# nekopanda/Amatsukaze

Measured on NVIDIA H100. Metric: 1920x1080i YV12 frames/sec (logo-eval + combing), higher is better.
Workload: dtype u8+f32

## Files before the change

amatsukaze_b200/csrc/amtk_b200.cu:

```cuda
#include "amtk_internal.h"
#include "logo_kernels.cuh"
#include "comb_kernels.cuh"
#include "comb_stream.cuh"
#include "comb_mma.cuh"
#include "scan_kernels.cuh"
#include "tnr_kernels.cuh"
#include <algorithm>
#include <cfloat>
#include <cmath>
#include <cstdlib>
#include <cstring>
#include <deque>
#include <memory>
#include <mutex>
#include <type_traits>

extern "C" { static int logo_ensure_device(const amtk_logo* cl, amtk_ctx* ctx, bool need_tables); }

namespace amtk {

static thread_local std::string g_error;
static constexpr size_t kEvalSmemLimit = 226 * 1024;
void set_error(const std::string& msg) { g_error = msg; }
bool cuda_ok(cudaError_t e, const char* what) {
// ... 272 lines not shown
          job.scores, count, countPad, n, sp.nfades, hl.blackScore, sp.take_abs, sum_out, out_frame_stride, sp.out_off, sp.out_fade_stride, rows);
    } else {
      logo_sum_kernel<<<(total + kSumThreads - 1) / kSumThreads, kSumThreads, 0, st>>>(
          job.scores, count, countPad, n, sp.nfades, hl.blackScore, sp.take_abs, sum_out, out_frame_stride, sp.out_off, sp.out_fade_stride, rows);
    }
    AMTK_CUDA(cudaGetLastError());
    ctx->launches += 2;
  }
  return 1;
}

static bool roi_inside(const amtk::HostLogo& full, const amtk_clip* clip, int pitch_elems) {
  if (full.imgx < 0 || full.imgy < 0) return false;
  const long long last = (long long)full.imgx + full.w - 1 + (long long)(full.imgy + full.h - 1) * pitch_elems;
  const long long plane_elems = (long long)clip->pitch_y / clip->bytes_per_sample * clip->height;
  return full.imgx + full.w <= pitch_elems && last < plane_elems;
}

static int comb_thresholds_ok(const amtk_comb_params* p, int bytes_per_sample) {
  if (bytes_per_sample == 2) {
    const int all[6] = { p->th_move_y, p->th_shima_y, p->th_lshima_y, p->th_move_c, p->th_shima_c, p->th_lshima_c };
    for (int v : all) if (v < 1) { set_error("comb: thresholds must be >= 1"); return 0; }
    if (p->th_move_y > 32768 || p->th_move_c > 32768) { set_error("comb: th_move must be in [1,32768] for 16-bit samples"); return 0; }
    return 1;
  }
  const int m[2] = { p->th_move_y, p->th_move_c };
  const int s[4] = { p->th_shima_y, p->th_lshima_y, p->th_shima_c, p->th_lshima_c };
  for (int v : m) if (v < 1 || v > 128) { set_error("comb: th_move must be in [1,128]"); return 0; }
  for (int v : s) if (v < 1 || v > 2047) { set_error("comb: th_shima/th_lshima must be in [1,2047]"); return 0; }
  return 1;
}

struct CombVariant {
  int R, strip, stages, sync, TH, boxH, threads, smem;
  void (*kernel)(const CombArgs);
  void (*kernel16)(const CombArgs);
};
template <typename Cfg> static CombVariant make_variant() {
  return CombVariant{ Cfg::R, Cfg::STRIP, Cfg::STAGES, Cfg::SYNC, Cfg::TH, Cfg::BOXH, Cfg::THREADS, Cfg::SMEM, comb_tma_kernel<Cfg, 1>, nullptr };
}
template <typename Cfg> static CombVariant make_variant16() {
  return CombVariant{ Cfg::R, Cfg::STRIP, Cfg::STAGES, Cfg::SYNC, Cfg::TH, Cfg::BOXH, Cfg::THREADS, Cfg::SMEM, comb_tma_kernel<Cfg, 1>, comb_tma_kernel<Cfg, 2> };
}
static const CombVariant* comb_variants(int* n) {
  static const CombVariant v[] = {
    make_variant16<CombCfg<15, 8, 3, 0>>(), make_variant16<CombCfg<16, 8, 3, 0>>(), make_variant16<CombCfg<17, 8, 3, 0>>(),
    make_variant<CombCfg<17, 8, 2, 0>>(), make_variant<CombCfg<17, 8, 4, 0>>(), make_variant<CombCfg<17, 8, 3, 1>>(),
  };
  *n = (int)(sizeof(v) / sizeof(v[0]));
  return v;
}

static int pick_comb_R(int hY, int hC) {
  int best = 16; long long best_waste = -1;
  for (int R = 17; R >= 15; --R) {
    const int th = 8 * R;
    const long long waste = (long long)((hY + th - 1) / th) * th - hY + 2LL * (((hC + th - 1) / th) * th - hC) / 2;
    if (best_waste < 0 || waste < best_waste) { best_waste = waste; best = R; }
  }
  return best;
}

struct WsVariant { int R, stages, warps, bps, TH, boxH, smem; bool band; void (*kernel)(const WsArgs); };
template <typename Cfg> static WsVariant make_ws() { return WsVariant{ Cfg::R, Cfg::STAGES, Cfg::WARPS, Cfg::BPS, Cfg::TH, Cfg::BOXH, Cfg::SMEM, Cfg::BAND, comb_ws_kernel<Cfg> }; }
static const WsVariant* ws_variants(int* n) {
  static const WsVariant v[] = { make_ws<WsCfg<17, 2>>(), make_ws<WsCfg<15, 2>>(), make_ws<WsCfg<16, 2>>(), make_ws<WsCfg<9, 2>>(), make_ws<WsCfg<15, 3>>(), make_ws<WsCfg<12, 2>>(), make_ws<WsCfg<10, 2>>(),
                                 make_ws<WsCfg<15, 2, 7>>(), make_ws<WsCfg<13, 2, 5>>(), make_ws<WsCfg<15, 2, 2>>(), make_ws<WsCfg<15, 3, 3>>(),
                                 make_ws<WsCfg<15, 2, 4, 2>>(), make_ws<WsCfg<16, 2, 4, 2>>(), make_ws<WsCfg<17, 2, 4, 2>>(),
                                 make_ws<WbCfg<15, 2>>(), make_ws<WbCfg<16, 2>>(), make_ws<WbCfg<17, 2>>(), make_ws<WbCfg<15, 3>>(),
                                 make_ws<WtCfg<15, 2>>(), make_ws<WtCfg<16, 2>>() };
  *n = (int)(sizeof(v) / sizeof(v[0]));
  return v;
}
static int pick_ws_R(int hY, int hC, int runs = kWsRuns) {
  int best = 17; long long best_waste = -1;
  for (int R : { 17, 16, 15 }) {
    const int th = runs * R;
    const long long waste = 2LL * ((long long)((hY + th - 1) / th) * th - hY) + 2LL * ((long long)((hC + th - 1) / th) * th - hC);
    if (best_waste < 0 || waste < best_waste) { best_waste = waste; best = R; }
  }
  return best;
}

static int ws_watchdog_ok(amtk_ctx* ctx) {
  if (!ctx->watch_pending) return 1;
  AMTK_CUDA(cudaEventSynchronize(ctx->ev_watch));
  ctx->watch_pending = false;
  const int* d = ctx->ws_watch;
  if (d[0]) {
    char msg[256];
    snprintf(msg, sizeof(msg), "comb_ws (band form): a device-side wait of the previous launch timed out (wait %d, step %d, CTA %d, thread %d, parity %d); its counters are not valid",
             d[1], d[2], d[3], d[4], d[5]);
    AMTK_FAIL(msg);
  }
  return 1;
}

static const int* ws_watch_record(const amtk_ctx* ctx) {
  return ctx->plan.dev.at<const int>(ctx->plan.q_off) + 16;
}

static CUtensorMapL2promotion comb_l2_promotion(const amtk_ctx* ctx) {
  switch (ctx->knobs.comb_l2) {
    case 0: return CU_TENSOR_MAP_L2_PROMOTION_NONE;
    case 64: return CU_TENSOR_MAP_L2_PROMOTION_L2_64B;
    case 256: return CU_TENSOR_MAP_L2_PROMOTION_L2_256B;
    default: return CU_TENSOR_MAP_L2_PROMOTION_L2_128B;
  }
}

template <typename Launch>
static int comb_launch(amtk_ctx* ctx, int* counts, int nf, Launch launch) {
  AMTK_CUDA(cudaMemsetAsync(counts, 0, (size_t)nf * 12 * sizeof(int), ctx->stream));
  std::pair<EventHandle, EventHandle> ev;
  if (ctx->timing) {
    if (!ctx->timing_pool.empty()) { ev = std::move(ctx->timing_pool.back()); ctx->timing_pool.pop_back(); }
    else { AMTK_CUDA(cudaEventCreate(ev.first.put())); AMTK_CUDA(cudaEventCreate(ev.second.put())); }
    AMTK_CUDA(cudaEventRecord(ev.first, ctx->stream));
  }
  launch();
  AMTK_CUDA(cudaGetLastError());
  if (ctx->timing) { AMTK_CUDA(cudaEventRecord(ev.second, ctx->stream)); ctx->timing_events.push_back(std::move(ev)); }
  ctx->launches += 1;
  return 1;
}

static_assert(std::has_unique_object_representations<amtk_ctx::CombPlanKey>::value, "plan keys are compared with memcmp");

template <typename Build>
static int comb_plan(amtk_ctx* ctx, const amtk_ctx::CombPlanKey& key, WsArgs& args, Build build) {
  amtk_ctx::CombPlan& plan = ctx->plan;
  if (!plan.valid || memcmp(&plan.key, &key, sizeof(key)) != 0) {
    const std::vector<CombSegment> segs = build();
    const size_t seg_bytes = segs.size() * sizeof(CombSegment);
    plan.q_off = (seg_bytes + 255) & ~(size_t)255;
    plan.valid = false;
    if (!plan.dev.ensure(plan.q_off + 256)) return 0;
    AMTK_CUDA(cudaMemcpyAsync(plan.dev.at(), segs.data(), seg_bytes, cudaMemcpyHostToDevice, ctx->stream));
    AMTK_CUDA(cudaStreamSynchronize(ctx->stream));
    plan.nitems = (int)segs.size(); plan.key = key; plan.valid = true;
  }
  AMTK_CUDA(cudaMemsetAsync(plan.dev.at(plan.q_off), 0, 256, ctx->stream));
  args.segs = plan.dev.at<const CombSegment>();
  args.nitems = plan.nitems;
  args.queue = plan.dev.at<int>(plan.q_off);
  return 1;
}

static const WsVariant* ws_variant(const amtk_ctx* ctx, const amtk_clip* clip, bool tall = true) {
  const int hY = clip->height, hC = clip->height >> clip->log_uvy;
  int nvar = 0; const WsVariant* vars = ws_variants(&nvar);
  const int bps = clip->bytes_per_sample;
  const bool band = bps == 1 && ctx->knobs.comb_ws_band && ctx->knobs.comb_ws_warps == kWsWarps;
  auto find = [&](int runs, int warps) -> const WsVariant* {
    const int R = ctx->knobs.comb_R ? ctx->knobs.comb_R : pick_ws_R(hY, hC, runs);
    for (int i = 0; i < nvar; ++i)
      if (vars[i].R == R && vars[i].stages == ctx->knobs.comb_ws_stages && vars[i].warps == warps && vars[i].bps == bps && vars[i].band == band) return &vars[i];
    return nullptr;
  };
  if (band && tall && ctx->knobs.comb_ws_band == 2)
    if (const WsVariant* V = find(kWtGroups * kWsRuns, kWtGroups * kWsWarps)) return V;
  return find(kWsRuns, ctx->knobs.comb_ws_warps);
}

static int launch_comb_ws(amtk_ctx* ctx, const amtk_clip* clip, const Window& win, int lo, int hi,
                          const amtk_comb_params* prm, int* dcounts, int out_row0, const ScanItemJob* lj = nullptr) {
  const int hY = clip->height, hC = clip->height >> clip->log_uvy;
  const int wY = clip->width, wC = clip->width >> clip->log_uvx;
  const int bps = clip->bytes_per_sample;
  const WsVariant* V = ws_variant(ctx, clip);
  if (!V) AMTK_FAIL("comb: no warp-stream kernel variant for the requested AMTK_COMB_* settings");
  const bool band = V->band;
  if (lj && !band) AMTK_FAIL("comb: logo items need the band form");
  const int WW = V->warps;
  if (!ws_watchdog_ok(ctx)) return 0;
  WsArgs args;
  memset(&args, 0, sizeof(args));
  const CUtensorMapL2promotion promo = comb_l2_promotion(ctx);
  for (int pl = 0; pl < 3; ++pl) {
    const long long off = pl == 0 ? 0 : (pl == 1 ? clip->off_u : clip->off_v);
    cuuint64_t gdim[3] = { (cuuint64_t)(pl ? wC : wY) * bps, (cuuint64_t)(pl ? hC : hY), (cuuint64_t)win.count };
    cuuint64_t gstr[2] = { (cuuint64_t)(pl ? clip->pitch_uv : clip->pitch_y), (cuuint64_t)clip->frame_stride };
    cuuint32_t box[3] = { (cuuint32_t)(band ? kWbHalf : kWsTW), (cuuint32_t)V->boxH, 1u };
    if (encode_map(ctx, &args.map[pl], CU_TENSOR_MAP_DATA_TYPE_UINT8, 3, win.dev_base + off, gdim, gstr, box, CU_TENSOR_MAP_SWIZZLE_NONE, promo) != CUDA_SUCCESS)
      AMTK_FAIL("cuTensorMapEncodeTiled failed");
  }
  const int remC = (wC * bps) % kWsTW;
  const long long uv_dist = clip->off_v - clip->off_u;
  const bool pair_uv = !band && ctx->knobs.comb_merge_uv && remC > 0 && remC <= kWsTW / 2 && uv_dist > 0 && (uv_dist & 15) == 0;
  if (pair_uv) {
    cuuint64_t gdim[4] = { (cuuint64_t)wC * bps, 2u, (cuuint64_t)hC, (cuuint64_t)win.count };
    cuuint64_t gstr[3] = { (cuuint64_t)uv_dist, (cuuint64_t)clip->pitch_uv, (cuuint64_t)clip->frame_stride };
    cuuint32_t box[4] = { (cuuint32_t)(kWsTW / 2), 2u, (cuuint32_t)V->boxH, 1u };
    if (encode_map(ctx, &args.map_uv, CU_TENSOR_MAP_DATA_TYPE_UINT8, 4, win.dev_base + clip->off_u, gdim, gstr, box, CU_TENSOR_MAP_SWIZZLE_NONE, promo) != CUDA_SUCCESS)
      AMTK_FAIL("cuTensorMapEncodeTiled(uv pair) failed");
  }
  const int tyY = (hY + V->TH - 1) / V->TH, tyC = (hC + V->TH - 1) / V->TH;
  int tile0 = 0, nc = 0;
  auto thresholds = [&](WsClass& C, bool chroma) {
    C.cls = chroma ? 1 : 0; C.H = chroma ? hC : hY;
    const int tM = chroma ? prm->th_move_c : prm->th_move_y, tS = chroma ? prm->th_shima_c : prm->th_shima_y, tL = chroma ? prm->th_lshima_c : prm->th_lshima_y;
    if (bps == 1) {
      C.thM = (unsigned)(0x80 - tM) * 0x01010101u;
      C.thS = (unsigned)tS * 0x00010001u;
      C.thL = (unsigned)tL * 0x00010001u;
    } else {
      C.thM = (unsigned)std::min(tM, 2047) * 0x00010001u;
      C.thS = (unsigned)(8192 + std::min(tS, 8191)) * 0x00010001u;
      C.thL = (unsigned)(8192 + std::min(tL, 8191)) * 0x00010001u;
    }
  };
  for (int pl = 0; pl < 3; ++pl) {
    WsClass& C = args.cl[nc];
    const int w = (pl ? wC : wY) * bps;
    C.kind = 0; C.map = pl; C.W = w; thresholds(C, pl != 0);
    C.tilesX = band ? (w + kWbW - 1) / kWbW : (pl && pair_uv) ? w / kWsTW : (w + kWsTW - 1) / kWsTW;
    C.tile0 = tile0; C.ntiles = C.tilesX * (pl ? tyC : tyY);
    if (C.ntiles == 0) continue;
    tile0 += C.ntiles; ++nc;
  }
  if (pair_uv) {
    WsClass& C = args.cl[nc];
    C.kind = 1; C.x0 = wC * bps - remC; C.tilesX = 1; thresholds(C, true);
    C.tile0 = tile0; C.ntiles = tyC; tile0 += C.ntiles; ++nc;
  }
  args.nclasses = nc;
  const int ntiles = tile0, nf = hi - lo;
  amtk_ctx::CombPlan& plan = ctx->plan;
  if (plan.occ_kernel != (const void*)V->kernel) {
    int occ = 0;
    AMTK_CUDA(cudaFuncSetAttribute(V->kernel, cudaFuncAttributeMaxDynamicSharedMemorySize, V->smem));
    AMTK_CUDA(cudaOccupancyMaxActiveBlocksPerMultiprocessor(&occ, V->kernel, 32 * WW, V->smem));
    if (occ < 1) AMTK_FAIL("comb kernel does not fit on an SM");
    plan.occ = occ; plan.occ_kernel = (const void*)V->kernel;
  }
  int occ = plan.occ;
  if (ctx->knobs.comb_ctas > 0) occ = std::min(occ, ctx->knobs.comb_ctas);
  const int logoF = lj ? lj->frames : 0, nlogo = lj ? (nf + logoF - 1) / logoF : 0;
  const long long total = (long long)ntiles * nf + nlogo;
  const int per_cta = band ? 1 : WW;
  const int nwarps = ctx->sm_count * occ * per_cta;
  const int grid = (int)std::min<long long>((long long)ctx->sm_count * occ, (total + per_cta - 1) / per_cta);
  const int f0 = lo - win.first;
  const amtk_ctx::CombPlanKey key{ (const void*)V->kernel, wY, hY, wC, hC, ntiles, nf, f0, ctx->knobs.comb_item, ctx->knobs.comb_tail,
                                   occ * WW, nlogo, logoF };
  if (!comb_plan(ctx, key, args, [&] {
    int big = ctx->knobs.comb_item > 0 ? ctx->knobs.comb_item : 64, small = std::max(4, big / 4);
    while (big > 8 && (long long)ntiles * (nf / big) < 6LL * nwarps) { big /= 2; small = std::max(4, big / 4); }
    const int tail_frames = std::min(nf, std::max(small, (int)(nf * 0.15)));
    const int head_frames = nf - tail_frames;
    const int tiny = ctx->knobs.comb_tail;
    const int end_frames = (tiny > 0 && tiny < small) ? std::min(tail_frames, std::max(tiny, (int)(nf * 0.04))) : 0;
    const int mid_end = nf - end_frames;
    std::vector<CombSegment> segs;
    segs.reserve((size_t)ntiles * (head_frames / big + tail_frames / small + (tiny > 0 ? end_frames / tiny : 0) + 3) + nlogo);
    auto tier = [&](int fa, int fz, int step) {
      if (band) {
        for (int f = fa; f < fz; f += step)
          for (int t = 0; t < ntiles; ++t) segs.push_back(CombSegment{ t, f0 + f, f0 + std::min(fz, f + step) });
      } else {
        for (int t = 0; t < ntiles; ++t)
          for (int f = fa; f < fz; f += step) segs.push_back(CombSegment{ t, f0 + f, f0 + std::min(fz, f + step) });
      }
    };
    tier(0, head_frames, big);
    if (nlogo > 0) {
      const std::vector<CombSegment> head(segs);
      const long long nhead = (long long)head.size();
      segs.clear();
      int k = 0;
      for (long long i = 0; i <= nhead; ++i) {
        for (; k < nlogo && (2LL * k + 1) * nhead / (2LL * nlogo) <= i; ++k)
          segs.push_back(CombSegment{ -1, f0 + k * logoF, f0 + std::min(nf, (k + 1) * logoF) });
        if (i < nhead) segs.push_back(head[(size_t)i]);
      }
    }
    tier(head_frames, mid_end, small);
    if (tiny > 0) tier(mid_end, nf, tiny);
    return segs;
  }))
    return 0;
  args.counts = dcounts;
  args.out_frame0 = out_row0 - win.first;
  args.prefetch = ctx->knobs.comb_ws_prefetch;
  if (lj) args.logo = *lj;
  if (!comb_launch(ctx, dcounts + (size_t)(lo - out_row0) * 12, nf, [&] { V->kernel<<<grid, 32 * WW, V->smem, ctx->stream>>>(args); }))
    return 0;
  if (band) {
    if (!ctx->ws_watch) {
      AMTK_CUDA(cudaHostAlloc(ctx->ws_watch.put(), 8 * sizeof(int), cudaHostAllocDefault));
      AMTK_CUDA(cudaEventCreateWithFlags(ctx->ev_watch.put(), cudaEventDisableTiming));
    }
    AMTK_CUDA(cudaMemcpyAsync(ctx->ws_watch, ws_watch_record(ctx), 8 * sizeof(int), cudaMemcpyDeviceToHost, ctx->stream));
    AMTK_CUDA(cudaEventRecord(ctx->ev_watch, ctx->stream));
    ctx->watch_pending = true;
  }
  return 1;
}

static int launch_comb_mma(amtk_ctx* ctx, const amtk_clip* clip, const Window& win, int lo, int hi,
                           const amtk_comb_params* prm, int* dcounts, int out_row0) {
  const int hY = clip->height, hC = clip->height >> clip->log_uvy;
  const int wY = clip->width, wC = clip->width >> clip->log_uvx;
  WsArgs args;
  memset(&args, 0, sizeof(args));
  for (int pl = 0; pl < 3; ++pl) {
    const long long off = pl == 0 ? 0 : (pl == 1 ? clip->off_u : clip->off_v);
    cuuint64_t gdim[3] = { (cuuint64_t)(pl ? wC : wY), (cuuint64_t)(pl ? hC : hY), (cuuint64_t)win.count };
    cuuint64_t gstr[2] = { (cuuint64_t)(pl ? clip->pitch_uv : clip->pitch_y), (cuuint64_t)clip->frame_stride };
    cuuint32_t box[3] = { (cuuint32_t)kMmTW, (cuuint32_t)kMmBoxH, 1u };
    if (encode_map(ctx, &args.map[pl], CU_TENSOR_MAP_DATA_TYPE_UINT8, 3, win.dev_base + off, gdim, gstr, box, CU_TENSOR_MAP_SWIZZLE_128B,
                   comb_l2_promotion(ctx)) != CUDA_SUCCESS)
      AMTK_FAIL("cuTensorMapEncodeTiled failed");
  }
  const int tyY = (hY + kMmTH - 1) / kMmTH, tyC = (hC + kMmTH - 1) / kMmTH;
  int tile0 = 0, nc = 0;
  for (int pl = 0; pl < 3; ++pl) {
    WsClass& C = args.cl[nc];
    const bool chroma = pl != 0;
    C.kind = 0; C.map = pl; C.cls = chroma ? 1 : 0; C.H = chroma ? hC : hY;
    C.thM = (unsigned)(0x80 - (chroma ? prm->th_move_c : prm->th_move_y)) * 0x01010101u;
    C.thS = (unsigned)(chroma ? prm->th_shima_c : prm->th_shima_y) * 0x00010001u;
    C.thL = (unsigned)(chroma ? prm->th_lshima_c : prm->th_lshima_y) * 0x00010001u;
    C.tilesX = ((chroma ? wC : wY) + kMmTW - 1) / kMmTW;
    C.tile0 = tile0; C.ntiles = C.tilesX * (chroma ? tyC : tyY);
    if (C.ntiles == 0) continue;
    tile0 += C.ntiles; ++nc;
  }
  args.nclasses = nc;
  const int ntiles = tile0, nf = hi - lo;
  amtk_ctx::CombPlan& plan = ctx->plan;
  const int NS = ctx->knobs.comb_mma == 2 ? 2 : 1;
  void (*kern)(const WsArgs) = NS == 2 ? comb_mma_kernel<2> : comb_mma_kernel<1>;
  const int smem = NS * kMmSmemPerStream + kMmBandBytes + 1024;
  if (plan.occ_kernel != (const void*)kern) {
    AMTK_CUDA(cudaFuncSetAttribute(kern, cudaFuncAttributeMaxDynamicSharedMemorySize, smem));
    int occ_q = 0;
    AMTK_CUDA(cudaOccupancyMaxActiveBlocksPerMultiprocessor(&occ_q, kern, kMmThreads, smem));
    if (occ_q < 1) AMTK_FAIL("comb_mma: kernel does not fit on an SM");
    plan.occ = occ_q; plan.occ_kernel = (const void*)kern;
  }
  int occ = plan.occ;
  if (ctx->knobs.comb_ctas > 0) occ = std::min(occ, ctx->knobs.comb_ctas);
  const int npairs_t = (ntiles + NS - 1) / NS;
  const long long total = (long long)npairs_t * nf;
  const int nstreams = ctx->sm_count * occ;
  const int grid = (int)std::min<long long>(nstreams, total);
  const int f0 = lo - win.first;
  const amtk_ctx::CombPlanKey key{ (const void*)kern, wY, hY, wC, hC, ntiles, nf, f0, ctx->knobs.comb_item, 0, occ, 0, 0 };
  if (!comb_plan(ctx, key, args, [&] {
    int big = ctx->knobs.comb_item > 0 ? ctx->knobs.comb_item : 64, small = std::max(4, big / 4);
    while (big > 8 && (long long)npairs_t * (nf / big) < 6LL * nstreams) { big /= 2; small = std::max(4, big / 4); }
    const int tail_frames = std::min(nf, std::max(small, (int)(nf * 0.15)));
    const int head_frames = nf - tail_frames;
    std::vector<CombSegment> segs;
    segs.reserve((size_t)NS * npairs_t * (head_frames / big + tail_frames / small + 2));
    auto push_block = [&](int fa, int fz) {
      for (int t = 0; t < ntiles; t += NS) {
        segs.push_back(CombSegment{ t, fa, fz });
        if (NS == 2) segs.push_back(CombSegment{ t + 1 < ntiles ? t + 1 : ~t, fa, fz });
      }
    };
    for (int f = 0; f < head_frames; f += big) push_block(f0 + f, f0 + std::min(head_frames, f + big));
    for (int f = head_frames; f < nf; f += small) push_block(f0 + f, f0 + std::min(nf, f + small));
    return segs;
  }))
    return 0;
  args.counts = dcounts;
  args.out_frame0 = out_row0 - win.first;
  if (!comb_launch(ctx, dcounts + (size_t)(lo - out_row0) * 12, nf, [&] { kern<<<grid, kMmThreads, smem, ctx->stream>>>(args); }))
    return 0;
  int dbg[8] = { 0, 0, 0, 0, 0, 0, 0, 0 };
  AMTK_CUDA(cudaMemcpyAsync(dbg, args.queue + 16, sizeof(dbg), cudaMemcpyDeviceToHost, ctx->stream));
  AMTK_CUDA(cudaStreamSynchronize(ctx->stream));
  if (dbg[0]) {
    char msg[256];
    snprintf(msg, sizeof(msg), "comb_mma<%d>: a device-side wait timed out (wait %d, step %d, CTA %d, thread %d, parity %d); results discarded",
             NS, dbg[1], dbg[2], dbg[3], dbg[4], dbg[5]);
    AMTK_FAIL(msg);
  }
// ... 840 lines not shown
  if (!(ctx->knobs.eval_par && n <= 16 && ctx->side_stream && ctx->side_stream2))
    return launch_eval(ctx, clip, win, lo, hi, pitch, sp, dout, 33, row0, ctx->stream, 0, frame_list) &&
           launch_eval(ctx, clip, win, lo, hi, pitch, st, dout, 33, row0, ctx->stream, 0, frame_list) &&
           launch_eval(ctx, clip, win, lo, hi, pitch, sb, dout, 33, row0, ctx->stream, 0, frame_list);
  const EvalSpec* specs[3] = { &sp, &st, &sb };
  size_t off[3], total = 0;
  for (int i = 0; i < 3; ++i) {
    if (!logo_ensure_device(specs[i]->logo, ctx, true)) return 0;
    off[i] = total;
    total += (((size_t)n * 11 * specs[i]->logo->countPad * sizeof(float)) + 255) & ~(size_t)255;
  }
  if (!ctx->scratch.ensure(total)) return 0;
  cudaStream_t streams[3] = { ctx->stream, ctx->side_stream, ctx->side_stream2 };
  cudaEvent_t joins[3] = { nullptr, ctx->ev_join1, ctx->ev_join2 };
  AMTK_CUDA(cudaEventRecord(ctx->ev_fork, ctx->stream));
  int ok = 1;
  for (int i = 0; i < 3 && ok; ++i) {
    if (i) ok = cuda_ok(cudaStreamWaitEvent(streams[i], ctx->ev_fork, 0), "cudaStreamWaitEvent");
    ok = ok && launch_eval(ctx, clip, win, lo, hi, pitch, *specs[i], dout, 33, row0, streams[i], off[i], frame_list);
    if (i && ok) ok = cuda_ok(cudaEventRecord(joins[i], streams[i]), "cudaEventRecord") &&
                      cuda_ok(cudaStreamWaitEvent(ctx->stream, joins[i], 0), "cudaStreamWaitEvent");
  }
  if (!ok) { cudaStreamSynchronize(ctx->side_stream); cudaStreamSynchronize(ctx->side_stream2); }
  return ok;
}

int amtk_logo_analyze_frames(amtk_ctx* ctx, const amtk_clip* clip, const amtk_logo* dl, const amtk_logo* ft, const amtk_logo* fb,
                             int frame0, int nframes, float* out, int out_on_device) {
  if (ctx && nframes == 0) return 1;
  if (!ctx || !dl || !ft || !fb || !out) AMTK_FAIL("amtk_logo_analyze_frames: bad argument");
  if (!validate_clip(clip, false)) return 0;
  if (ft->host.w != dl->host.w || fb->host.w != dl->host.w || ft->host.h != dl->host.h / 2 || fb->host.h != dl->host.h / 2)
    AMTK_FAIL("field logos do not match the deint logo");
  DevSelect ds(ctx); if (!ds.ok) return 0;
  const size_t bytes = (size_t)nframes * 33 * sizeof(float);
  float* d = out;
  if (!out_on_device) { d = host_out_buffer(ctx, bytes); if (!d) return 0; }
  if (!roi_inside(dl->host, clip, clip->pitch_y / clip->bytes_per_sample)) AMTK_FAIL("logo rectangle lies outside the frame");
  if (!for_each_roi_window(ctx, clip, frame0, nframes, dl->host.imgx, dl->host.imgy, dl->host.w, dl->host.h, false, false,
                           [&](const amtk_clip& v, const Window& w, int lo, int hi, int dx, int dy) {
        return analyze_impl(ctx, &v, dx, dy, dl, ft, fb, w, lo, hi, d, frame0); }))
    return 0;
  return finish_output(ctx, out, d, bytes, out_on_device);
}

int amtk_logo_eval_fades(amtk_ctx* ctx, const amtk_clip* clip, const amtk_logo* dl, const float* fades, int nfades,
                         int frame0, int nframes, float* out, int out_on_device) {
  if (ctx && nframes == 0) return 1;
  if (!ctx || !dl || !fades || !out) AMTK_FAIL("amtk_logo_eval_fades: bad argument");
  if (nfades < 1 || nfades > kMaxFades) AMTK_FAIL("amtk_logo_eval_fades: 1..24 fade levels");
  if (!validate_clip(clip, false)) return 0;
  DevSelect ds(ctx); if (!ds.ok) return 0;
  const size_t bytes = (size_t)nframes * nfades * sizeof(float);
  float* d = out;
  if (!out_on_device) { d = host_out_buffer(ctx, bytes); if (!d) return 0; }
  const int pitch = clip->pitch_y / clip->bytes_per_sample;
  if (!roi_inside(dl->host, clip, pitch)) AMTK_FAIL("logo rectangle lies outside the frame");
  if (!for_each_roi_window(ctx, clip, frame0, nframes, dl->host.imgx, dl->host.imgy, dl->host.w, dl->host.h, false, false,
                           [&](const amtk_clip& v, const Window& w, int lo, int hi, int dx, int dy) {
        EvalSpec sp{ dl, dl->host.imgx - dx, dl->host.imgy - dy, dl->host.w, dl->host.h, 0, 0, dl->host.w, nfades, fades, 0, 0, 1 };
        return launch_eval(ctx, &v, w, lo, hi, v.pitch_y / v.bytes_per_sample, sp, d, nfades, frame0, ctx->stream, 0); }))
    return 0;
  return finish_output(ctx, out, d, bytes, out_on_device);
}

void amtk_comb_default_params(amtk_comb_params* p) {
  if (!p) return;
  p->th_move_y = 20; p->th_shima_y = 12; p->th_lshima_y = 36;
  p->th_move_c = 24; p->th_shima_c = 16; p->th_lshima_c = 48;
}

int amtk_comb_frames(amtk_ctx* ctx, const amtk_clip* clip, const amtk_comb_params* prm, int frame0, int nframes,
                     int32_t* counts, int out_on_device) {
  if (ctx && nframes == 0) return 1;
  if (!ctx || !prm || !counts) AMTK_FAIL("amtk_comb_frames: bad argument");
  if (!validate_clip(clip, true) || !comb_thresholds_ok(prm, clip->bytes_per_sample)) return 0;
  DevSelect ds(ctx); if (!ds.ok) return 0;
  const size_t bytes = (size_t)nframes * 12 * sizeof(int32_t);
  int* d = counts;
  if (!out_on_device) { if (!ctx->dout2.ensure(bytes)) return 0; d = ctx->dout2.at<int>(); }
  if (!for_each_window(ctx, clip, frame0, nframes, true, [&](const Window& w, int lo, int hi) {
        return launch_comb(ctx, clip, w, lo, hi, prm, d, frame0); }))
    return 0;
  return finish_output(ctx, counts, d, bytes, out_on_device);
}

static int scan_item_frames(const amtk_logo* lg, const amtk_ctx* ctx, const amtk_clip* clip) {
  const WsVariant* V = ws_variant(ctx, clip, false);
  if (!V) return 0;
  const size_t ring = (size_t)V->smem - 128;
  int F = 0;
  while (F < kScanItemMaxFrames && scan_item_smem_bytes(lg->host.w, lg->host.h, lg->countPad, F + 1) <= ring) ++F;
  return F;
}

int amtk_scan_comb_frames(amtk_ctx* ctx, const amtk_clip* clip, amtk_logo* const* logos, int nlogos,
                          const amtk_comb_params* prm, int frame0, int nframes, float* scores, int32_t* counts, int out_on_device) {
  if (ctx && nframes == 0) return 1;
  if (!ctx || !prm || !counts || !scores || !logos || nlogos < 1) AMTK_FAIL("amtk_scan_comb_frames: bad argument");
  if (!validate_clip(clip, true) || !comb_thresholds_ok(prm, clip->bytes_per_sample)) return 0;
  DevSelect ds(ctx); if (!ds.ok) return 0;
  const size_t sbytes = (size_t)nframes * nlogos * 2 * sizeof(float), cbytes = (size_t)nframes * 12 * sizeof(int32_t);
  float* ds_ = scores; int* dc = counts;
  if (!out_on_device) {
    if (!ctx->dout.ensure(sbytes) || !ctx->dout2.ensure(cbytes)) return 0;
    ds_ = ctx->dout.at<float>(); dc = ctx->dout2.at<int>();
  }
  const amtk_logo* lg0 = logos[0];
  const bool one_logo = nlogos == 1 && lg0 && lg0->has_mask && lg0->host.count() > 0 &&
                        lg0->host.imgw == clip->width && lg0->host.imgh == clip->height && lg0->host.imgx >= 0 && lg0->host.imgy >= 0 &&
                        lg0->host.imgx + lg0->host.w <= clip->width && lg0->host.imgy + lg0->host.h <= clip->height;
  if (!for_each_window(ctx, clip, frame0, nframes, true, [&](const Window& w, int lo, int hi) -> int {
        const WsVariant* V = one_logo && comb_runs_band(ctx, clip, w) ? ws_variant(ctx, clip) : nullptr;
        const int F = V ? scan_item_frames(lg0, ctx, clip) : 0;
        if (F > 0) {
          if (!logo_ensure_device(lg0, ctx, true)) return 0;
          ScanItemJob lj;
          lj.ybase = w.dev_base; lj.frame_stride = clip->frame_stride; lj.pitch = clip->pitch_y;
          lj.imgx = lg0->host.imgx; lj.imgy = lg0->host.imgy;
          lj.logo = logo_dev(lg0); lj.maxv = (float)((1 << clip->bits_per_sample) - 1);
          lj.frames = F; lj.scores = ds_;
          return launch_comb_ws(ctx, clip, w, lo, hi, prm, dc, frame0, &lj);
        }
        return launch_comb(ctx, clip, w, lo, hi, prm, dc, frame0) &&
               scan_frames_impl(ctx, clip, clip, 0, 0, logos, nlogos, w, lo, hi, 0, ds_, frame0); }))
    return 0;
  if (out_on_device) return 1;
  AMTK_CUDA(cudaMemcpyAsync(scores, ds_, sbytes, cudaMemcpyDeviceToHost, ctx->stream));
  AMTK_CUDA(cudaMemcpyAsync(counts, dc, cbytes, cudaMemcpyDeviceToHost, ctx->stream));
  AMTK_CUDA(cudaStreamSynchronize(ctx->stream));
  return 1;
}

static int scan_sample_bits(const amtk_clip* c) {
  if (c->bytes_per_sample == 1) {
    if (c->bits_per_sample <= 8) return 8;
  } else if (c->bits_per_sample > 8 && c->bits_per_sample <= 16) {
    if (((c->pitch_y | c->pitch_uv | c->off_u | c->off_v | c->frame_stride | (int64_t)reinterpret_cast<uintptr_t>(c->base)) & 1) == 0)
      return c->bits_per_sample;
    set_error("LogoScan: 2-byte clips need even pitches, plane offsets, frame stride and base");
    return 0;
  }
  set_error("LogoScan: bits_per_sample must be at most 8 for 1-byte samples and 9..16 for 2-byte samples");
  return 0;
}

int amtk_scan_create(amtk_ctx* ctx, int scanw, int scanh, int lx, int ly, int thy, amtk_scan** out) {
  if (!ctx || !out) AMTK_FAIL("amtk_scan_create: null argument");
  if (scanw < 4 || scanh < 4 || scanw > 4096 || scanh > 4096 || lx < 0 || lx > 2 || ly < 0 || ly > 2) AMTK_FAIL("amtk_scan_create: bad geometry");
  DevSelect ds(ctx); if (!ds.ok) return 0;
  std::unique_ptr<amtk_scan> s(new amtk_scan());
  s->ctx = ctx; s->device = ctx->device; s->scanw = scanw; s->scanh = scanh; s->logUVx = lx; s->logUVy = ly; s->thy = thy;
  s->npix = (size_t)scanw * scanh + 2 * (size_t)(scanw >> lx) * (scanh >> ly);
  if (!cuda_ok(cudaMalloc(s->dSums.put(), s->npix * 3 * sizeof(unsigned long long)), "cudaMalloc") ||
      !cuda_ok(cudaMalloc(s->dBg.put(), 8 * sizeof(unsigned long long)), "cudaMalloc") ||
      !cuda_ok(cudaMemsetAsync(s->dSums, 0, s->npix * 3 * sizeof(unsigned long long), ctx->stream), "cudaMemsetAsync") ||
      !cuda_ok(cudaMemsetAsync(s->dBg, 0, 8 * sizeof(unsigned long long), ctx->stream), "cudaMemsetAsync"))
    return 0;
  *out = s.release();
  return 1;
}

void amtk_scan_destroy(amtk_scan* s) {
  if (!s) return;
  DevSelect ds(s->device);
  delete s;
}

int amtk_scan_add_frames(amtk_scan* s, const amtk_clip* clip, int scanx, int scany, int frame0, int nframes,
                         const uint8_t* frame_select, uint8_t* valid_out) {
  if (!s) AMTK_FAIL("amtk_scan_add_frames: null scan");
  amtk_ctx* ctx = s->ctx;
  if (!validate_clip(clip, true)) return 0;
  const int bits = scan_sample_bits(clip);
  if (!bits) return 0;
  if (s->bytes_per_sample && (clip->bytes_per_sample != s->bytes_per_sample || bits != s->bits))
    AMTK_FAIL("LogoScan: the clip's sample format differs from the first clip's");
  if (clip->log_uvx != s->logUVx || clip->log_uvy != s->logUVy) AMTK_FAIL("chroma subsampling mismatch");
  if (scanx < 0 || scany < 0 || scanx + s->scanw > clip->width || scany + s->scanh > clip->height) AMTK_FAIL("scan rectangle outside the frame");
  if (frame0 < 0 || nframes < 0 || frame0 + nframes > clip->num_frames) AMTK_FAIL("frame range outside the clip");
  DevSelect ds(ctx); if (!ds.ok) return 0;
  s->bytes_per_sample = clip->bytes_per_sample; s->bits = bits;
  const bool wide = clip->bytes_per_sample == 2;
  const size_t bg_bytes = (size_t)nframes * sizeof(int4), off_sel = (bg_bytes + 255) & ~(size_t)255;
  const size_t off_val = off_sel + (((size_t)nframes + 255) & ~(size_t)255);
  if (!ctx->dout.ensure(off_val + (size_t)nframes + 256)) return 0;
  uint8_t* base = ctx->dout.at();
  int4* dbg = reinterpret_cast<int4*>(base); uint8_t* dsel = base + off_sel; uint8_t* dval = base + off_val;
  if (frame_select) AMTK_CUDA(cudaMemcpyAsync(dsel, frame_select, (size_t)nframes, cudaMemcpyHostToDevice, ctx->stream));
  const int ok = for_each_roi_window(ctx, clip, frame0, nframes, scanx, scany, s->scanw, s->scanh, true, false,
                                     [&](const amtk_clip& v, const Window& w, int lo, int hi, int dx, int dy) {
    ScanClip c;
    c.base = w.dev_base; c.frame_stride = v.frame_stride; c.offU = v.off_u; c.offV = v.off_v;
    c.pitchY = v.pitch_y / v.bytes_per_sample; c.pitchUV = v.pitch_uv / v.bytes_per_sample;
    c.scanx = scanx - dx; c.scany = scany - dy; c.scanw = s->scanw; c.scanh = s->scanh; c.logUVx = s->logUVx; c.logUVy = s->logUVy; c.thy = s->thy;
    c.frame0 = lo - w.first; c.nframes = hi - lo;
    const int rel = lo - frame0;
    if (wide) scan_border16_kernel<<<hi - lo, 256, 0, ctx->stream>>>(c, frame_select ? dsel + rel : nullptr, dbg + rel);
    else scan_border_kernel<<<hi - lo, 256, 0, ctx->stream>>>(c, frame_select ? dsel + rel : nullptr, dbg + rel);
    AMTK_CUDA(cudaGetLastError());
    const int pixblocks = (int)((s->npix + 255) / 256);
    const int splits = std::max(1, std::min(hi - lo, (ctx->sm_count * 8) / pixblocks));
    if (wide) scan_accumulate16_kernel<<<dim3(pixblocks, splits), 256, 0, ctx->stream>>>(c, dbg + rel, s->dSums, s->dBg, dval + rel);
    else scan_accumulate_kernel<<<dim3(pixblocks, splits), 256, 0, ctx->stream>>>(c, dbg + rel, s->dSums, s->dBg, dval + rel);
    AMTK_CUDA(cudaGetLastError());
    ctx->launches += 2;
    return 1;
  });
  if (!ok) return 0;
  std::vector<uint8_t> tmp;
  unsigned long long nv = 0;
  if (valid_out) AMTK_CUDA(cudaMemcpyAsync(valid_out, dval, (size_t)nframes, cudaMemcpyDeviceToHost, ctx->stream));
  AMTK_CUDA(cudaMemcpyAsync(&nv, s->dBg + 6, sizeof(nv), cudaMemcpyDeviceToHost, ctx->stream));
  AMTK_CUDA(cudaStreamSynchronize(ctx->stream));
// ... 1266 lines not shown
```

amatsukaze_b200/csrc/amtk_internal.h:

```cpp
#pragma once
#include <cuda.h>
#include <cuda_runtime.h>
#include <algorithm>
#include <cstdint>
#include <cstdio>
#include <mutex>
#include <string>
#include <vector>
#include "../../include/amtk_b200.h"
#include "logo_host.h"

typedef CUresult (*amtk_encode_tiled_fn)(CUtensorMap*, CUtensorMapDataType, cuuint32_t, void*, const cuuint64_t*,
                                         const cuuint64_t*, const cuuint32_t*, const cuuint32_t*, CUtensorMapInterleave,
                                         CUtensorMapSwizzle, CUtensorMapL2promotion, CUtensorMapFloatOOBfill);

namespace amtk {

void set_error(const std::string& msg);
bool cuda_ok(cudaError_t e, const char* what);

#define AMTK_CUDA(call)                                          \
  do {                                                           \
    if (!::amtk::cuda_ok((call), #call)) return 0;               \
  } while (0)
// ... 23 lines not shown
using StreamHandle = CudaOwned<cudaStream_t, cudaStreamDestroy>;

struct GrowBuf {
  DevBuf<uint8_t> buf;
  size_t cap = 0;
  bool ensure(size_t need) {
    if (cap >= need) return true;
    buf.reset(); cap = 0;
    const size_t sz = std::max(need, (size_t)1 << 20);
    uint8_t* p = nullptr;
    if (!cuda_ok(cudaMalloc(&p, sz), "cudaMalloc(scratch)")) return false;
    buf.reset(p); cap = sz;
    return true;
  }
  template <class T = uint8_t> T* at(size_t byte_off = 0) const { return reinterpret_cast<T*>(buf.get() + byte_off); }
};

struct LogoDev {
  int w, h, count, countPad;
  float blackScore;
  const float* A;
  const float* B;
  const uint32_t* pix;
  const float* tapsT;
  const float2* scales;
};

}

struct amtk_ctx {
  mutable std::recursive_mutex mu;
  int device = 0;
  cudaStream_t stream = nullptr;
  amtk::StreamHandle owned_stream;
  amtk::StreamHandle copy_stream;
  amtk::StreamHandle side_stream, side_stream2;
  amtk::EventHandle ev_fork, ev_join1, ev_join2;
  amtk::EventHandle ev_copy[2];
  amtk::EventHandle ev_done[2];
  int sm_count = 0;
  int64_t launches = 0;
  long long h2d_bytes_last = 0;
  amtk::GrowBuf scratch;
  amtk::GrowBuf stage[2];
  amtk::GrowBuf small;
  amtk::GrowBuf dout;
  amtk::GrowBuf dout2;
  amtk::GrowBuf erase_clip;
  amtk::PinnedBuf<void> hout; void* hout_dev = nullptr;
  amtk_encode_tiled_fn encode_tiled = nullptr;
  struct Knobs {
    int eval_waves = 1;
    int eval_cw = 1;
    int eval_par = 1;
    int comb_generic = 0;
    int comb_merge_uv = 1;
    int comb_part = -1;
    int comb_strip = 8, comb_stages = 3, comb_R = 0, comb_ctas = 0, comb_sync = 0, comb_l2 = 64;
    int comb_item = 0;
    int comb_tail = 4;
    int comb_ws_stages = 2;
    int comb_mma = 0;
    int comb_ws10 = 0;
    int comb_ws_warps = 4;
    int comb_ws_prefetch = 0;
    int comb_ws_band = 2;
    int comb_ws = 1;
  } knobs;
  struct CombPlanKey {
    const void* kernel;
    int wY, hY, wC, hC, ntiles, nf, f0;
    int item, tail;
    int ctas;
    int nlogo, logoF;
  };
  struct CombPlan {
    bool valid = false;
    CombPlanKey key{};
    amtk::GrowBuf dev;
    int nitems = 0; size_t q_off = 0;
    int occ = 0; const void* occ_kernel = nullptr;
  } plan;
  amtk::PinnedBuf<int> ws_watch;
  amtk::EventHandle ev_watch;
  bool watch_pending = false;
  bool timing = false;
  std::vector<std::pair<amtk::EventHandle, amtk::EventHandle>> timing_events;
  std::vector<std::pair<amtk::EventHandle, amtk::EventHandle>> timing_pool;
  double timing_ms = 0.0; int64_t timing_count = 0;
};

struct amtk_logo {
  int device = -1;
  amtk::HostLogo host;
  amtk::DevBuf<float> dA, dB;
  amtk::DevBuf<float> dAU, dBU, dAV, dBV;
  amtk::DevBuf<uint32_t> dPix; amtk::DevBuf<float> dTapsT; amtk::DevBuf<float2> dScales;
  int countPad = 0;
  bool has_mask = false;
  bool tables_uploaded = false;
  std::mutex mu;
};

struct amtk_scan {
  amtk_ctx* ctx = nullptr;
  int device = 0;
  int scanw = 0, scanh = 0, logUVx = 1, logUVy = 1, thy = 0;
  int nvalid = 0;
  int bytes_per_sample = 0, bits = 0;
  amtk::DevBuf<unsigned long long> dSums;
  amtk::DevBuf<unsigned long long> dBg;
  size_t npix = 0;
};
```

amatsukaze_b200/csrc/logo_kernels.cuh:

```cuda
#pragma once
#include "amtk_internal.h"
#include "exact_math.h"
#include "tma_utils.cuh"

namespace amtk {

constexpr int kEvalThreads = 512;
constexpr int kMaxFades = 24;

struct EvalJob {
  const void* ybase;
  long long frame_stride;
  int pitch;
  int frame0, nframes;
  const int* frame_list;
  int list_base;
  int imgx, imgy;
  int roi_w, roi_h;
  int src_mode;
  int src_off, src_stride;
  LogoDev logo;
  float maxv;
  int nfades;
  float fades[kMaxFades];
// ... 83 lines not shown
      pixel_t* dst = reinterpret_cast<pixel_t*>(raw_base);
      int x = roi_x0, y = roi_y0;
      for (int i = tid; i < roi_n; i += kEvalThreads) {
        dst[x + y * raw_pitch] = roi[x + (long long)y * job.pitch];
        x += roi_dx; y += roi_dy; if (x >= roi_w) { x -= roi_w; ++y; }
      }
      __syncthreads();
      raw = dst;
    }
    {
      int x = roi_x0, y = roi_y0;
      for (int i = tid; i < roi_n; i += kEvalThreads) {
        const pixel_t* rp = raw + x + y * raw_pitch;
        float v;
        if (job.src_mode == 0 && y > 0 && y < roi_h - 1) {
          const int a = rp[-raw_pitch], b = rp[0], c = rp[raw_pitch];
          v = (float)(a + 2 * b + c + 2) / 4.0f;
        } else {
          v = (float)rp[0];
        }
        src[i] = v;
        x += roi_dx; y += roi_dy; if (x >= roi_w) { x -= roi_w; ++y; }
      }
    }
    __syncthreads();

    const int fstep = job.pair_fades ? 2 : 1;
    for (int fi = 0; fi < job.nfades; fi += fstep) {
      const int nf2 = min(fstep, job.nfades - fi);
      const float fade0 = job.fades[fi], fade1 = job.fades[fi + nf2 - 1];
      const float omf0 = AMTK_FSUB(1.0f, fade0), omf1 = AMTK_FSUB(1.0f, fade1);
      {
        int x = lg_x0, y = lg_y0;
        for (int i = tid; i < npx; i += kEvalThreads) {
          const float srcv = src[job.src_off + x + y * job.src_stride];
          const float av = sA[i], bv = sB[i];
          work[i] = remove_logo(srcv, av, bv, job.maxv, fade0, omf0);
          if (nf2 == 2) work2[i] = remove_logo(srcv, av, bv, job.maxv, fade1, omf1);
          x += lg_dx; y += lg_dy; if (x >= w) { x -= w; ++y; }
        }
      }
      __syncthreads();
      float* out0 = job.scores + ((size_t)f * job.nfades + fi) * lg.countPad;
      float sum[2][PXT]; int bin[2][PXT];
#pragma unroll
      for (int p = 0; p < PXT; ++p) {
        const float* wp = work + pxy[p];
        float avg;
        sum[0][p] = corr5x5_tree(taps[p], [&](int dy, int dx) { return wp[dy * w + dx]; }, &avg);
        bin[0][p] = scale_bin(avg);
        if (nf2 == 2) {
          const float* wq = work2 + pxy[p];
          sum[1][p] = corr5x5_tree(taps[p], [&](int dy, int dx) { return wq[dy * w + dx]; }, &avg);
          bin[1][p] = scale_bin(avg);
        }
      }
#pragma unroll
      for (int p = 0; p < PXT; ++p) {
        if (cidx[p] < lg.count) {
          const float2* sc = lg.scales + (size_t)cidx[p] * 32;
          const float2 s0 = __ldg(sc + bin[0][p]);
          out0[cidx[p]] = pixel_score(sum[0][p], s0.x, s0.y);
          if (nf2 == 2) {
            const float2 s1 = __ldg(sc + bin[1][p]);
            out0[lg.countPad + cidx[p]] = pixel_score(sum[1][p], s1.x, s1.y);
          }
        }
      }
      __syncthreads();
    }
  }
}

struct ScanItemJob {
  const uint8_t* ybase;
  long long frame_stride;
  int pitch;
  int imgx, imgy;
  LogoDev logo;
  float maxv;
  int frames;
  float* scores;
};
constexpr int kScanItemMaxFrames = 8;
__host__ __device__ inline size_t scan_item_smem_bytes(int w, int h, int countPad, int frames) {
  return (2 * (((size_t)w * h + 8 + 3) & ~(size_t)3) + (size_t)frames * 2 * (countPad + 4)) * sizeof(float) + (size_t)((w + 30) & ~15) * h;
}

__device__ __forceinline__ void cp_async16(void* smem_dst, const void* src) {
  asm volatile("cp.async.cg.shared.global [%0], [%1], 16;" ::"r"(smem_u32(smem_dst)), "l"(src) : "memory");
}
__device__ __forceinline__ void cp_async4(void* smem_dst, const void* src) {
  asm volatile("cp.async.ca.shared.global [%0], [%1], 4;" ::"r"(smem_u32(smem_dst)), "l"(src) : "memory");
}

template <int NT>
__device__ __forceinline__ void scan_item(const ScanItemJob& j, int fbegin, int fend, int out_frame0, uint8_t* smem) {
  const LogoDev& lg = j.logo;
  const int tid = threadIdx.x, w = lg.w, h = lg.h, npx = w * h, count = lg.count, spitch = lg.countPad + 4;
  float* work0 = reinterpret_cast<float*>(smem);
  float* work1 = work0 + ((npx + 8 + 3) & ~3);
  float* sc = work1 + ((npx + 8 + 3) & ~3);
  uint8_t* raw = reinterpret_cast<uint8_t*>(sc + (size_t)j.frames * 2 * spitch);
  const int xa = j.imgx & ~15, xo = j.imgx - xa;
  const int rpitch = (xo + w + 15) & ~15, cpr = rpitch >> 4, nchunks = cpr * h;
  const float omf0 = AMTK_FSUB(1.0f, 0.0f), omf1 = AMTK_FSUB(1.0f, 1.0f);
  const int dx = NT % w, dy = NT / w, y0 = tid / w, x0 = tid - y0 * w;
  for (int f = fbegin; f < fend; ++f) {
    __syncthreads();
    const uint8_t* roi = j.ybase + (long long)f * j.frame_stride + xa + (long long)j.imgy * j.pitch;
    for (int k = tid; k < nchunks; k += NT) {
      const int y = k / cpr;
      cp_async16(raw + 16 * k, roi + (long long)y * j.pitch + 16 * (k - y * cpr));
    }
    for (int q = tid; q < (npx >> 2); q += NT) { cp_async16(work0 + 4 * q, lg.A + 4 * q); cp_async16(work1 + 4 * q, lg.B + 4 * q); }
    for (int i = (npx & ~3) + tid; i < npx; i += NT) { cp_async4(work0 + i, lg.A + i); cp_async4(work1 + i, lg.B + i); }
    asm volatile("cp.async.wait_all;" ::: "memory");
    __syncthreads();
    {
      int x = x0, y = y0;
      for (int i = tid; i < npx; i += NT) {
        const uint8_t* rp = raw + y * rpitch + xo + x;
        float v;
        if (y > 0 && y < h - 1) { const int a = rp[-rpitch], b = rp[0], c = rp[rpitch]; v = (float)(a + 2 * b + c + 2) / 4.0f; }
        else v = (float)rp[0];
        const float av = work0[i], bv = work1[i];
        work0[i] = remove_logo(v, av, bv, j.maxv, 0.0f, omf0);
        work1[i] = remove_logo(v, av, bv, j.maxv, 1.0f, omf1);
        x += dx; y += dy; if (x >= w) { x -= w; ++y; }
      }
    }
    __syncthreads();
    float* s0 = sc + (size_t)(f - fbegin) * 2 * spitch;
    float2 kp0 = make_float2(0.0f, 0.0f), kp1 = kp0;
    int cp = -1;
#pragma unroll 1
    for (int c = tid; c < count; c += NT) {
      const uint32_t pv = __ldg(lg.pix + c);
      float taps[25];
#pragma unroll
      for (int t = 0; t < 25; ++t) taps[t] = __ldg(lg.tapsT + (size_t)t * lg.countPad + c);
      const int o = (int)((pv & 0xFFFFu) - 2) + (int)((pv >> 16) - 2) * w;
      float avg0, avg1;
      s0[c] = corr5x5_tree(taps, [&](int ry, int rx) { return work0[o + ry * w + rx]; }, &avg0);
      s0[spitch + c] = corr5x5_tree(taps, [&](int ry, int rx) { return work1[o + ry * w + rx]; }, &avg1);
      const float2 kn0 = __ldg(lg.scales + (size_t)c * 32 + scale_bin(avg0)), kn1 = __ldg(lg.scales + (size_t)c * 32 + scale_bin(avg1));
      if (cp >= 0) { s0[cp] = pixel_score(s0[cp], kp0.x, kp0.y); s0[spitch + cp] = pixel_score(s0[spitch + cp], kp1.x, kp1.y); }
      kp0 = kn0; kp1 = kn1; cp = c;
    }
    if (cp >= 0) { s0[cp] = pixel_score(s0[cp], kp0.x, kp0.y); s0[spitch + cp] = pixel_score(s0[spitch + cp], kp1.x, kp1.y); }
  }
  __syncthreads();
  if (tid < 2 * (fend - fbegin)) {
    const float* row = sc + (size_t)tid * spitch;
    const float4* row4 = reinterpret_cast<const float4*>(row);
    const int n4 = count >> 2;
    float r = 0.0f;
#pragma unroll 1
    for (int i = 0; i < n4; ++i) {
      const float4 v = row4[i];
      r = AMTK_FADD(r, v.x); r = AMTK_FADD(r, v.y); r = AMTK_FADD(r, v.z); r = AMTK_FADD(r, v.w);
    }
    for (int c = n4 << 2; c < count; ++c) r = AMTK_FADD(r, row[c]);
    j.scores[(size_t)(fbegin + (tid >> 1) - out_frame0) * 2 + (tid & 1)] = AMTK_FDIV(r, lg.blackScore);
  }
}

constexpr int kSumThreads = 32;
__global__ void __launch_bounds__(kSumThreads) logo_sum_kernel(const float* __restrict__ scores, int count, int countPad,
                                                               int nframes, int nfades, float blackScore, int take_abs,
                                                               float* __restrict__ out, int out_frame_stride, int out_off,
                                                               int out_fade_stride, const int* __restrict__ out_rows) {
  const int t = blockIdx.x * blockDim.x + threadIdx.x;
  if (t >= nframes * nfades) return;
  const float4* row = reinterpret_cast<const float4*>(scores + (size_t)t * countPad);
  const int nlines = countPad >> 5;
  float4 cur[8], nxt[8];
#pragma unroll
  for (int k = 0; k < 8; ++k) cur[k] = row[k];
  float r = 0.0f;
  int c = 0;
  for (int l = 0; l < nlines; ++l) {
    if (l + 1 < nlines) {
#pragma unroll
      for (int k = 0; k < 8; ++k) nxt[k] = row[(l + 1) * 8 + k];
    }
    if (c + 32 <= count) {
#pragma unroll
      for (int k = 0; k < 8; ++k) {
        r = AMTK_FADD(r, cur[k].x); r = AMTK_FADD(r, cur[k].y); r = AMTK_FADD(r, cur[k].z); r = AMTK_FADD(r, cur[k].w);
      }
      c += 32;
    } else {
#pragma unroll
      for (int k = 0; k < 8; ++k) {
        if (c < count) r = AMTK_FADD(r, cur[k].x); ++c;
        if (c < count) r = AMTK_FADD(r, cur[k].y); ++c;
        if (c < count) r = AMTK_FADD(r, cur[k].z); ++c;
        if (c < count) r = AMTK_FADD(r, cur[k].w); ++c;
      }
    }
#pragma unroll
    for (int k = 0; k < 8; ++k) cur[k] = nxt[k];
  }
  float v = AMTK_FDIV(r, blackScore);
  if (take_abs) v = fabsf(v);
  const int f = t / nfades, fi = t - f * nfades;
  out[(size_t)(out_rows ? out_rows[f] : f) * out_frame_stride + out_off + (size_t)fi * out_fade_stride] = v;
}

__global__ void __launch_bounds__(32) logo_sum_bulk_kernel(const float* __restrict__ scores, int count, int countPad,
                                                            int nframes, int nfades, float blackScore, int take_abs,
                                                            float* __restrict__ out, int out_frame_stride, int out_off,
                                                            int out_fade_stride, const int* __restrict__ out_rows) {
  extern __shared__ __align__(16) float sum_rows[];
  __shared__ __align__(8) uint64_t bar;
  const int lane = threadIdx.x, total = nframes * nfades;
  const int t0 = blockIdx.x * 32, nrows = min(32, total - t0);
  const int pitch = countPad + 4;
  const uint32_t row_bytes = (uint32_t)countPad * sizeof(float);
  if (lane == 0) { mbar_init(&bar, 1); asm volatile("fence.mbarrier_init.release.cluster;" ::: "memory"); }
  __syncwarp();
  if (lane == 0) mbar_expect_tx(&bar, row_bytes * (uint32_t)nrows);
  __syncwarp();
  if (lane < nrows) bulk_load_1d(sum_rows + (size_t)lane * pitch, scores + (size_t)(t0 + lane) * countPad, row_bytes, &bar);
  mbar_wait(&bar, 0);
  if (lane >= nrows) return;
  const float4* row = reinterpret_cast<const float4*>(sum_rows + (size_t)lane * pitch);
  float r = 0.0f;
  const int n4 = count >> 2;
#pragma unroll 8
  for (int i = 0; i < n4; ++i) {
    const float4 v = row[i];
    r = AMTK_FADD(r, v.x); r = AMTK_FADD(r, v.y); r = AMTK_FADD(r, v.z); r = AMTK_FADD(r, v.w);
  }
  const float* tail = sum_rows + (size_t)lane * pitch;
  for (int c = n4 << 2; c < count; ++c) r = AMTK_FADD(r, tail[c]);
  float v = AMTK_FDIV(r, blackScore);
  if (take_abs) v = fabsf(v);
  const int t = t0 + lane;
  const int f = t / nfades, fi = t - f * nfades;
  out[(size_t)(out_rows ? out_rows[f] : f) * out_frame_stride + out_off + (size_t)fi * out_fade_stride] = v;
}

__global__ void fill_pairs_kernel(float* out, int nframes, int stride, int off, float v0, float v1) {
  const int f = blockIdx.x * blockDim.x + threadIdx.x;
// ... 5 lines not shown
```

Baseline: 918,500.

## Double-buffer comb watchdog readback, raise logo frames per item, pipeline score reduction

The band-form watchdog record now uses two pinned slots and two events. A new launch only waits on the launch from two steps back, and the previous one is checked after the current launch is enqueued, instead of blocking on the prior launch before every encode. The maximum number of logo frames folded into one scan item rises from 8 to 16, sized against the band variant's shared memory. The per-row score sum now prefetches 8 float4 values ahead in registers. These aim to cut host-device serialisation and per-item overhead, at the cost of more shared memory per item and later error reporting.

```diff
diff --git a/amatsukaze_b200/csrc/amtk_b200.cu b/amatsukaze_b200/csrc/amtk_b200.cu
--- a/amatsukaze_b200/csrc/amtk_b200.cu
+++ b/amatsukaze_b200/csrc/amtk_b200.cu
@@ -378,18 +378,21 @@
   return best;
 }
 
-static int ws_watchdog_ok(amtk_ctx* ctx) {
-  if (!ctx->watch_pending) return 1;
-  AMTK_CUDA(cudaEventSynchronize(ctx->ev_watch));
-  ctx->watch_pending = false;
-  const int* d = ctx->ws_watch;
+static int ws_watchdog_ok(amtk_ctx* ctx, int k) {
+  if (!ctx->watch_pending[k]) return 1;
+  AMTK_CUDA(cudaEventSynchronize(ctx->ev_watch[k]));
+  ctx->watch_pending[k] = false;
+  const int* d = ctx->ws_watch + 8 * k;
   if (d[0]) {
     char msg[256];
-    snprintf(msg, sizeof(msg), "comb_ws (band form): a device-side wait of the previous launch timed out (wait %d, step %d, CTA %d, thread %d, parity %d); its counters are not valid",
+    snprintf(msg, sizeof(msg), "comb_ws (band form): a device-side wait timed out (wait %d, step %d, CTA %d, thread %d, parity %d); its counters are not valid",
              d[1], d[2], d[3], d[4], d[5]);
     AMTK_FAIL(msg);
   }
   return 1;
+}
+static int ws_watchdog_synced(amtk_ctx* ctx) {
+  return ws_watchdog_ok(ctx, ctx->watch_next) && ws_watchdog_ok(ctx, ctx->watch_next ^ 1);
 }
 
 static const int* ws_watch_record(const amtk_ctx* ctx) {
@@ -469,7 +472,8 @@
   const bool band = V->band;
   if (lj && !band) AMTK_FAIL("comb: logo items need the band form");
   const int WW = V->warps;
-  if (!ws_watchdog_ok(ctx)) return 0;
+  if (!ws_watchdog_ok(ctx, ctx->watch_next)) return 0;
+  const int prev = ctx->watch_next ^ 1;
   WsArgs args;
   memset(&args, 0, sizeof(args));
   const CUtensorMapL2promotion promo = comb_l2_promotion(ctx);
@@ -584,14 +588,16 @@
     return 0;
   if (band) {
     if (!ctx->ws_watch) {
-      AMTK_CUDA(cudaHostAlloc(ctx->ws_watch.put(), 8 * sizeof(int), cudaHostAllocDefault));
-      AMTK_CUDA(cudaEventCreateWithFlags(ctx->ev_watch.put(), cudaEventDisableTiming));
+      AMTK_CUDA(cudaHostAlloc(ctx->ws_watch.put(), 2 * 8 * sizeof(int), cudaHostAllocDefault));
+      for (EventHandle& e : ctx->ev_watch) AMTK_CUDA(cudaEventCreateWithFlags(e.put(), cudaEventDisableTiming));
     }
-    AMTK_CUDA(cudaMemcpyAsync(ctx->ws_watch, ws_watch_record(ctx), 8 * sizeof(int), cudaMemcpyDeviceToHost, ctx->stream));
-    AMTK_CUDA(cudaEventRecord(ctx->ev_watch, ctx->stream));
-    ctx->watch_pending = true;
-  }
-  return 1;
+    const int k = ctx->watch_next;
+    AMTK_CUDA(cudaMemcpyAsync(ctx->ws_watch + 8 * k, ws_watch_record(ctx), 8 * sizeof(int), cudaMemcpyDeviceToHost, ctx->stream));
+    AMTK_CUDA(cudaEventRecord(ctx->ev_watch[k], ctx->stream));
+    ctx->watch_pending[k] = true;
+    ctx->watch_next = k ^ 1;
+  }
+  return ws_watchdog_ok(ctx, prev);
 }
 
 static int launch_comb_mma(amtk_ctx* ctx, const amtk_clip* clip, const Window& win, int lo, int hi,
@@ -1598,15 +1604,17 @@
   if (!for_each_window(ctx, clip, frame0, nframes, true, [&](const Window& w, int lo, int hi) {
         return launch_comb(ctx, clip, w, lo, hi, prm, d, frame0); }))
     return 0;
-  return finish_output(ctx, counts, d, bytes, out_on_device);
+  return finish_output(ctx, counts, d, bytes, out_on_device) && (out_on_device || ws_watchdog_synced(ctx));
 }
 
 static int scan_item_frames(const amtk_logo* lg, const amtk_ctx* ctx, const amtk_clip* clip) {
-  const WsVariant* V = ws_variant(ctx, clip, false);
-  if (!V) return 0;
-  const size_t ring = (size_t)V->smem - 128;
+  const WsVariant* V4 = ws_variant(ctx, clip, false);
+  const WsVariant* V = ws_variant(ctx, clip);
+  if (!V4 || !V) return 0;
+  const int w = lg->host.w, h = lg->host.h;
+  if (scan_item_smem_bytes(w, h, lg->countPad, 1) > (size_t)V4->smem - 128) return 0;
   int F = 0;
-  while (F < kScanItemMaxFrames && scan_item_smem_bytes(lg->host.w, lg->host.h, lg->countPad, F + 1) <= ring) ++F;
+  while (F < kScanItemMaxFrames && scan_item_smem_bytes(w, h, lg->countPad, F + 1) <= (size_t)V->smem - 128) ++F;
   return F;
 }
 
@@ -1645,7 +1653,7 @@
   AMTK_CUDA(cudaMemcpyAsync(scores, ds_, sbytes, cudaMemcpyDeviceToHost, ctx->stream));
   AMTK_CUDA(cudaMemcpyAsync(counts, dc, cbytes, cudaMemcpyDeviceToHost, ctx->stream));
   AMTK_CUDA(cudaStreamSynchronize(ctx->stream));
-  return 1;
+  return ws_watchdog_synced(ctx);
 }
 
 static int scan_sample_bits(const amtk_clip* c) {
diff --git a/amatsukaze_b200/csrc/amtk_internal.h b/amatsukaze_b200/csrc/amtk_internal.h
--- a/amatsukaze_b200/csrc/amtk_internal.h
+++ b/amatsukaze_b200/csrc/amtk_internal.h
@@ -129,8 +129,9 @@
     int occ = 0; const void* occ_kernel = nullptr;
   } plan;
   amtk::PinnedBuf<int> ws_watch;
-  amtk::EventHandle ev_watch;
-  bool watch_pending = false;
+  amtk::EventHandle ev_watch[2];
+  bool watch_pending[2] = { false, false };
+  int watch_next = 0;
   bool timing = false;
   std::vector<std::pair<amtk::EventHandle, amtk::EventHandle>> timing_events;
   std::vector<std::pair<amtk::EventHandle, amtk::EventHandle>> timing_pool;
diff --git a/amatsukaze_b200/csrc/logo_kernels.cuh b/amatsukaze_b200/csrc/logo_kernels.cuh
--- a/amatsukaze_b200/csrc/logo_kernels.cuh
+++ b/amatsukaze_b200/csrc/logo_kernels.cuh
@@ -189,7 +189,7 @@
   int frames;
   float* scores;
 };
-constexpr int kScanItemMaxFrames = 8;
+constexpr int kScanItemMaxFrames = 16;
 __host__ __device__ inline size_t scan_item_smem_bytes(int w, int h, int countPad, int frames) {
   return (2 * (((size_t)w * h + 8 + 3) & ~(size_t)3) + (size_t)frames * 2 * (countPad + 4)) * sizeof(float) + (size_t)((w + 30) & ~15) * h;
 }
@@ -259,16 +259,30 @@
   }
   __syncthreads();
   if (tid < 2 * (fend - fbegin)) {
-    const float* row = sc + (size_t)tid * spitch;
-    const float4* row4 = reinterpret_cast<const float4*>(row);
-    const int n4 = count >> 2;
+    const float4* row = reinterpret_cast<const float4*>(sc + (size_t)tid * spitch);
+    const int nlines = lg.countPad >> 5;
+    float4 q[8];
+#pragma unroll
+    for (int k = 0; k < 8; ++k) q[k] = row[k];
     float r = 0.0f;
+    int c = 0;
 #pragma unroll 1
-    for (int i = 0; i < n4; ++i) {
-      const float4 v = row4[i];
-      r = AMTK_FADD(r, v.x); r = AMTK_FADD(r, v.y); r = AMTK_FADD(r, v.z); r = AMTK_FADD(r, v.w);
-    }
-    for (int c = n4 << 2; c < count; ++c) r = AMTK_FADD(r, row[c]);
+    for (int l = 0; l < nlines; ++l) {
+      const bool more = l + 1 < nlines;
+#pragma unroll
+      for (int k = 0; k < 8; ++k) {
+        const float4 v = q[k];
+        if (more) q[k] = row[(l + 1) * 8 + k];
+        if (c + 4 <= count) {
+          r = AMTK_FADD(r, v.x); r = AMTK_FADD(r, v.y); r = AMTK_FADD(r, v.z); r = AMTK_FADD(r, v.w);
+        } else {
+          if (c < count) r = AMTK_FADD(r, v.x);
+          if (c + 1 < count) r = AMTK_FADD(r, v.y);
+          if (c + 2 < count) r = AMTK_FADD(r, v.z);
+        }
+        c += 4;
+      }
+    }
     j.scores[(size_t)(fbegin + (tid >> 1) - out_frame0) * 2 + (tid & 1)] = AMTK_FDIV(r, lg.blackScore);
   }
 }
```

Result: faster. 949,300, median of 6 (+3.4%).
